# winddori2002/DEX-TTS

Measured on AMD Instinct MI355X. Metric: mel-frames/s at n_timesteps=50, 80-ch mel (sampler only); RTF, higher is better.
Workload: dtype bf16; 1 GPU; gedex_b1: gedex_lj B=1/GPU T=512 n_timesteps=50 (BASELINE.json configs[1]); global_batch=1, frames=512, hipgraph=False, parallelism=1 GPU

## Files before the change

### dex_tts_amd/csrc/dex_api.hip

```cpp
#include <hip/hip_runtime.h>
#include <cstdlib>

#include <cmath>
#include <cstdarg>
#include <atomic>
#include <cstdio>
#include <mutex>
#include <cstring>
#include <map>
#include <unordered_map>
#include <string_view>
#include <string>
#include <vector>

#include "../../include/dex_amd.h"
#include "kernels.h"
#include "weight_store.h"

using namespace dex;

namespace dex {
namespace {
const char* const KNOB_NAMES[] = {
    "DEX_CONV_STREAM", "DEX_CONV_PP", "DEX_CONV_SKIP_DEAD", "DEX_H_BF16", "DEX_ATTN_SEPARATE", "DEX_ATTN_Q64", "DEX_ATTN_Q64_TAIL", "DEX_ATTN_Q64_HALF", "DEX_DIT_XCDS", "DEX_ATTN_GENERIC", "DEX_RES2", "DEX_LP_INTER", "DEX_DIT_CHAIN",
    "DEX_DIT_CLUSTER", "DEX_DIT_CLUSTER_LOCAL", "DEX_ATTN_X_LP", "DEX_RES_X_LP", "DEX_CAT_LP", "DEX_XCD_MAP", "DEX_DEBUG_DROP_HANDOFF", "DEX_PATCH_FUSED",
    "DEX_CONV_DOWN", "DEX_CONVT_UP", "DEX_DEBUG_PLAN",
    "DEX_ATTN_SHARED_W8", "DEX_CONVT_MT", "DEX_CONVT_WGS", "DEX_CONV_DOWN_WGS", "DEX_CONV_REGW", "DEX_CONV_REGW_RES", "DEX_CONV_SMALL_MAX", "DEX_CONV_TH8",
    "DEX_CONV_W8", "DEX_DWCONV_CAP", "DEX_FINAL_CAP", "DEX_FIRST_CAP", "DEX_FIRST_MFMA", "DEX_GEMM_NWALK", "DEX_NWALK_SPLIT", "DEX_NWALK_BM", "DEX_POS_COL", "DEX_POS_COL_MIN",
    "DEX_POS_CT", "DEX_REGW_MIN_TILES", "DEX_REGW_WGS", "DEX_ROWCHAIN64", "DEX_ROWCHAIN64A", "DEX_TIV_CAP", "DEX_TV_CHAIN", "DEX_TIV_FOLD", "DEX_LINATTN_NSUB", "DEX_TV_FOLD", "DEX_OUT2_MIN", "DEX_NWALK_DMA",
    "DEX_LINATTN_HEADWAVES", "DEX_LINATTN_OUT2_HW", "DEX_CONV_ROUND1", "DEX_CONV_RESIDENT", "DEX_KVCTX_ROWS", "DEX_OUT2_ROWS", "DEX_PE_TOK", "DEX_NWALK_SMALL"};
constexpr int N_KNOBS = (int)(sizeof(KNOB_NAMES) / sizeof(KNOB_NAMES[0]));
int knob_parse(const char* e) {
    if (!e) return KNOB_UNSET;
    char* end = nullptr;
    const long v = strtol(e, &end, 10);
    if (end == e) {
        static bool warned = false;
        if (!warned) { warned = true; fprintf(stderr, "libdexamd: ignoring a DEX_* knob whose value '%s' is not an integer\n", e); }
        return KNOB_UNSET;
    }
    return (int)v;
}
struct KnobSnapshot {
    int v[N_KNOBS];
    KnobSnapshot() { for (int i = 0; i < N_KNOBS; ++i) v[i] = knob_parse(getenv(KNOB_NAMES[i])); }
};
thread_local const KnobSnapshot* t_knobs = nullptr;
struct WsplitScope {
    bool prev;
    explicit WsplitScope(bool on) : prev(g_lp_wsplit) { g_lp_wsplit = on; }
    ~WsplitScope() { g_lp_wsplit = prev; }
};
struct KnobScope {
    const KnobSnapshot* prev;
    explicit KnobScope(const KnobSnapshot* k) : prev(t_knobs) { t_knobs = k; }
    ~KnobScope() { t_knobs = prev; }
};
}
static int knob_index(const char* name) {
    static const std::unordered_map<std::string_view, int> idx = [] {
        std::unordered_map<std::string_view, int> m;
        for (int i = 0; i < N_KNOBS; ++i) m.emplace(KNOB_NAMES[i], i);
        return m;
    }();
    const auto it = idx.find(std::string_view(name));
    return it == idx.end() ? -1 : it->second;
}
int knob(const char* name) {
    if (t_knobs) {
        const int i = knob_index(name);
        if (i >= 0) return t_knobs->v[i];
    }
    return knob_parse(getenv(name));
}
}
static_assert(PREC_FP32 == DEX_PREC_FP32 && PREC_BF16 == DEX_PREC_BF16 && PREC_FP16 == DEX_PREC_FP16 && PREC_FP16X2 == DEX_PREC_FP16X2, "kernels.h mirrors DexPrecision");

namespace {
void xcd_map_probe();

struct TD { float* p; int ld; int coff; int C; int lp = 0; };

struct ResW { PackedW w1, w2, wr; const float *b1, *g1, *be1, *b2, *g2, *be2, *br, *mlp_w, *mlp_b; int cin, cout; };
constexpr int ATT_KSPLIT_MAX = 4;
static int att_split_cap(long tokens) { return tokens <= 20480 ? 8 : ATT_KSPLIT_MAX; }
static bool attention_q64_regime(int N, int B) {
    if (N < 1024) return dit_sep64_small_n(N, B) && dit_rowchain64_form(N, B, 0);
    const int ks = attention_q64_ksplit(N, B, att_split_cap((long)B * N));
    const int nt32 = (N + 31) / 32, ng = (nt32 + 7) / 8;
    return 2L * B * ng * ks >= 128;
}
struct LinW { PackedW wqkv; const float *wqkv_raw, *wout_raw, *bias_eff, *g; LpView wkv[3], wq_frag[3]; int C; };
struct DitBlockW { PackedW wqkv, wproj, wfc1, wfc2; const float *bqkv, *bproj, *bfc1, *bfc2, *ada_w, *ada_b; };

struct Prof { std::string name; hipEvent_t a, b; double flops, bytes; };
struct ProfAgg { std::string name; int calls; double ms, flops, bytes; };

struct Arena {
    char* base = nullptr; size_t off = 0, cap = 0; bool dry = true;
    void* take(size_t bytes) {
        off = (off + 255) & ~size_t(255);
        void* p = dry ? nullptr : (void*)(base + off);
        if (!dry && trace) fprintf(stderr, "plan[%d] off %zu bytes %zu\n", trace++, off, bytes);
        off += bytes;
        return p;
    }
    int trace = 0;
    float* f(size_t n) { return (float*)take(n * sizeof(float)); }
};

}

struct DexCtx : WeightStore {
    DexCtx() : WeightStore("") {}
    DexConfig cfg{};
    int lpi() const { return precision == DEX_PREC_FP16X2 ? 2 : precision == DEX_PREC_FP16 ? 1 : 0; }
    int lp_kind() const { return precision == DEX_PREC_BF16 ? 1 : 2; }
    bool lp() const { return precision != DEX_PREC_FP32; }
    bool tuned = true;
    int precision = DEX_PREC_FP32;
    std::vector<std::vector<ResW>> down_res, up_res;
    std::vector<LinW> down_lin, up_lin;
    std::vector<PackedW> down_ds_w;
    std::vector<std::vector<PackedW>> up_us_w;
    std::vector<const float*> down_ds_b, up_us_b;
    const float *fc_w3 = nullptr, *fc_w1 = nullptr;
    PackedW fin_w, pe_pw, fl_w, tv_wk, tv_wv, tv_wl;
    PackedW pos_w;
    const float *fin_b = nullptr, *fin_g = nullptr, *fin_be = nullptr, *fconv_w = nullptr, *fconv_b = nullptr;
    const float *pe_dw = nullptr, *pe_db = nullptr, *pe_pb = nullptr, *pos_b = nullptr, *freq_pos = nullptr;
    std::vector<DitBlockW> blocks;
    const float *fl_b = nullptr, *fl_ada_w = nullptr, *fl_ada_b = nullptr;
    const float *tv_wq_raw = nullptr;
    float *mel_basis = nullptr, *mel_filt = nullptr; void* mel_ws = nullptr; size_t mel_ws_bytes = 0;
    const int* last_xerr = nullptr;
    int* st_host = nullptr; hipEvent_t st_ev = nullptr; bool st_pending = false;
    struct Tap { std::string name; const float* p; std::vector<int64_t> shape; };
    std::vector<Tap> taps;
    bool prof_on = false;
    std::vector<Prof> prof;
    std::vector<ProfAgg> prof_agg;
    struct GraphEntry { std::vector<uint64_t> key; hipGraphExec_t exec; uint64_t stamp; const int* xerr; };
    std::vector<GraphEntry> graphs;
    uint64_t graph_clock = 0;
    void drop_graphs() { for (auto& g : graphs) hipGraphExecDestroy(g.exec); graphs.clear(); }
    template <typename F> int replay(const std::vector<uint64_t>& key, hipStream_t st, F&& enqueue);
    void reset_records() {
        taps.clear();
        if (prof_on) { for (auto& pr : prof) { hipEventDestroy(pr.a); hipEventDestroy(pr.b); } prof.clear(); prof_agg.clear(); }
    }
};

template <typename F> int DexCtx::replay(const std::vector<uint64_t>& key, hipStream_t st, F&& enqueue) {
    GraphEntry* hit = nullptr;
    for (auto& g : graphs) if (g.key == key) { hit = &g; break; }
    if (!hit) {
        constexpr size_t MAX_GRAPHS = 8;
        if (graphs.size() >= MAX_GRAPHS) {
            size_t lru = 0;
            for (size_t i = 1; i < graphs.size(); ++i) if (graphs[i].stamp < graphs[lru].stamp) lru = i;
            hipGraphExecDestroy(graphs[lru].exec);
            graphs.erase(graphs.begin() + lru);
        }
        hipGraph_t graph = nullptr;
        DEX_HIPCHK(this, hipStreamBeginCapture(st, hipStreamCaptureModeThreadLocal));
        const int rc = enqueue();
        hipError_t ec = hipStreamEndCapture(st, &graph);
        if (rc) { if (graph) hipGraphDestroy(graph); return rc; }
        if (ec != hipSuccess || !graph) return fail(DEX_ERR_HIP, "stream capture failed: %s", hipGetErrorString(ec));
        hipGraphExec_t exec = nullptr;
        ec = hipGraphInstantiate(&exec, graph, nullptr, nullptr, 0);
        hipGraphDestroy(graph);
        if (ec != hipSuccess) return fail(DEX_ERR_HIP, "hipGraphInstantiate failed: %s", hipGetErrorString(ec));
        graphs.push_back({key, exec, 0, last_xerr});
        hit = &graphs.back();
    }
    last_xerr = hit->xerr;
    hit->stamp = ++graph_clock;
// ... 1763 lines not shown
```

### dex_tts_amd/csrc/dit_rowchain.hip

```cpp
#include <hip/hip_runtime.h>
#include "kernels.h"
#include <cstdlib>
#include "lp_util.h"
#include "kernels_lp.h"

namespace dex {
namespace DEX_LP_NS {

typedef float f32x16 __attribute__((ext_vector_type(16)));
typedef unsigned short u16;

namespace {

constexpr int RC_H = 256, RC_MLP = 512, RC_ROWS = 32, RC_NW = 8;
constexpr int A_LD = RC_H + 8;
constexpr int H_LD = RC_MLP + 8;
constexpr int X_LD = RC_H + 4;
constexpr int AT_LD = 132;
constexpr size_t RC_LDS_ATTN = (size_t)(RC_NW * 32 * AT_LD + RC_NW * 64) * sizeof(float);
constexpr size_t RC_LDS = (size_t)RC_ROWS * (A_LD + H_LD) * sizeof(u16) + (size_t)RC_ROWS * X_LD * sizeof(float) + 4 * RC_H * sizeof(float);

__device__ __forceinline__ float gelu_erf_rc(float x) {
    const float z = fabsf(x) * 0.70710678118654752440f;
    const float t = __builtin_amdgcn_rcpf(fmaf(0.3275911f, z, 1.0f));
// ... 803 lines not shown
    {
        float4 v[4]; bool ok[4];
#pragma unroll
        for (int k = 0; k < 4; ++k) {
            const int row = wave + 4 * k;
            const bool need_q = row >= 10 || row == 2 || row == 3;
            ok[k] = row < 13 && (need_q ? has_q : !p.qkv_only);
            const float* src = !ok[k] ? ada
                             : row == 0 ? ada + 3 * RC_H : row == 1 ? ada + 4 * RC_H
                             : row == 2 ? p.next_shift + (long)step * p.next_step_stride
                             : row == 3 ? p.next_scale + (long)step * p.next_step_stride
                             : row == 4 ? ada + 2 * RC_H : row == 5 ? p.bp : row == 6 ? ada + 5 * RC_H : row == 7 ? p.b2
                             : row < 10 ? p.b1 + (row - 8) * RC_H : p.bq + (row - 10) * RC_H;
            v[k] = reinterpret_cast<const float4*>(src)[tid & 63];
        }
#pragma unroll
        for (int k = 0; k < 4; ++k) {
            const int row = wave + 4 * k;
            if (row == 1 || row == 3) { v[k].x += 1.f; v[k].y += 1.f; v[k].z += 1.f; v[k].w += 1.f; }
            if (ok[k]) reinterpret_cast<float4*>(PRM + row * RC_H)[tid & 63] = v[k];
        }
    }
    for (;;) {
        const int next = tile + (int)gridDim.x;
        const bool more = next < ntiles;
        RCA_DESC(, tile, true)
        RCA_DESC(_n, more ? next : tile, more)
        const long hb = ((long)b * 2 + (wave >> 1)) * p.Npad * 256;
        const int hsz = has_q ? p.Npad * 256 : 0;
        const auto rq = __builtin_amdgcn_make_buffer_rsrc(reinterpret_cast<unsigned char*>(p.Qh) + hb, 0, hsz, 0x00020000);
        const auto rk = __builtin_amdgcn_make_buffer_rsrc(reinterpret_cast<unsigned char*>(p.Kh) + hb, 0, hsz, 0x00020000);
        const auto rv = __builtin_amdgcn_make_buffer_rsrc(reinterpret_cast<unsigned char*>(p.Vt) + hb, 0, hsz, 0x00020000);
        const long long* dbg = p.dbg ? p.dbg + ((long)tile * 4 + wave) * 32 : nullptr;
#ifdef RCA_TIMING
        if (dbg && (tid & 63) == 0) const_cast<long long*>(dbg)[31] = tile == (int)blockIdx.x ? t_entry : 0;
#endif
        if (p.qkv_only) { asm volatile(RCA_ASM_QKV RCA_OPERANDS); }
        else if (has_q) { asm volatile(RCA_ASM_FULL RCA_OPERANDS); }
        else { asm volatile(RCA_ASM_LAST RCA_OPERANDS); }
        if (!more) break;
        tile = next;
    }
#undef RCA_OPERANDS
#undef RCA_DESC
}

namespace {
constexpr int CL_AH_LD = 128 + 8;
constexpr int CL_RED_LD = 33;
typedef unsigned u32x4v __attribute__((ext_vector_type(4)));

__device__ __forceinline__ void wload8(WT8& w, const void* W, long lo_u4, int ksteps_total, int nt, int ks0, int lane) {
    const uint4* src = reinterpret_cast<const uint4*>(W) + ((long)nt * ksteps_total + ks0) * 64 + lane;
#pragma unroll
    for (int j = 0; j < 8; ++j) w.h[j] = src[j * 64];
#ifdef DEX_LP_WSPLIT
#pragma unroll
    for (int j = 0; j < 8; ++j) w.l[j] = src[lo_u4 + j * 64];
#endif
    __builtin_amdgcn_sched_barrier(0);
}
__device__ __forceinline__ void mma8(f32x16& acc, const WT8& w, const u16* a_lane) {
    u32x4 a[8];
#pragma unroll
    for (int j = 0; j < 8; ++j) a[j] = *reinterpret_cast<const u32x4*>(a_lane + j * 16);
    __builtin_amdgcn_sched_barrier(0);
#pragma unroll
    for (int j = 0; j < 8; ++j) acc = DEX_MFMA_LP(__builtin_bit_cast(lp8, a[j]), __builtin_bit_cast(lp8, w.h[j]), acc, 0, 0, 0);
#ifdef DEX_LP_WSPLIT
#pragma unroll
    for (int j = 0; j < 8; ++j) acc = DEX_MFMA_LP(__builtin_bit_cast(lp8, a[j]), __builtin_bit_cast(lp8, w.l[j]), acc, 0, 0, 0);
#endif
}
__device__ __forceinline__ void ln_regs_to_A(float4 (&v)[4], u16* As, const float* shift, const float* scale, int row, int seg) {
    float4 sc[4], sh[4];
#pragma unroll
    for (int q = 0; q < 4; ++q) {
        sc[q] = *reinterpret_cast<const float4*>(scale + q * 64 + seg * 4);
        sh[q] = *reinterpret_cast<const float4*>(shift + q * 64 + seg * 4);
    }
    float s = 0.f;
#pragma unroll
    for (int q = 0; q < 4; ++q) s += (v[q].x + v[q].y) + (v[q].z + v[q].w);
#pragma unroll
    for (int o = 1; o < 16; o <<= 1) s += __shfl_xor(s, o);
    const float mean = s * (1.f / RC_H);
    float ss = 0.f;
#pragma unroll
    for (int q = 0; q < 4; ++q) {
        v[q].x -= mean; v[q].y -= mean; v[q].z -= mean; v[q].w -= mean;
        ss += v[q].x * v[q].x + v[q].y * v[q].y + v[q].z * v[q].z + v[q].w * v[q].w;
    }
#pragma unroll
    for (int o = 1; o < 16; o <<= 1) ss += __shfl_xor(ss, o);
    const float rstd = rsqrtf(ss * (1.f / RC_H) + 1e-6f);
#pragma unroll
    for (int q = 0; q < 4; ++q) {
        uint2 o;
        o.x = pack2_lp(v[q].x * rstd * (1.f + sc[q].x) + sh[q].x, v[q].y * rstd * (1.f + sc[q].y) + sh[q].y);
        o.y = pack2_lp(v[q].z * rstd * (1.f + sc[q].z) + sh[q].z, v[q].w * rstd * (1.f + sc[q].w) + sh[q].w);
        *reinterpret_cast<uint2*>(As + row * A_LD + q * 64 + seg * 4) = o;
    }
}
template <bool LOCAL> struct ClScope {
    static constexpr int ST_AUX = LOCAL ? 0 : 16, LD_AUX = LOCAL ? 1 : 16;
    static __device__ __forceinline__ unsigned poll(unsigned* p) {
        if constexpr (LOCAL) {
            unsigned v;
            asm volatile("global_atomic_or %0, %1, %2, off sc0\n\ts_waitcnt vmcnt(0)" : "=v"(v) : "v"(p), "v"(0u) : "memory");
            return v;
        } else return __hip_atomic_load(p, __ATOMIC_RELAXED, __HIP_MEMORY_SCOPE_AGENT);
    }
    static __device__ __forceinline__ void st(unsigned* p, unsigned v) {
        if constexpr (LOCAL) __hip_atomic_store(p, v, __ATOMIC_RELAXED, __HIP_MEMORY_SCOPE_WORKGROUP);
        else __hip_atomic_store(p, v, __ATOMIC_RELAXED, __HIP_MEMORY_SCOPE_AGENT);
    }
    static __device__ __forceinline__ unsigned long long ld64(const unsigned long long* p) {
        if constexpr (LOCAL) return __hip_atomic_load(p, __ATOMIC_RELAXED, __HIP_MEMORY_SCOPE_WORKGROUP);
        else return __hip_atomic_load(p, __ATOMIC_RELAXED, __HIP_MEMORY_SCOPE_AGENT);
    }
    static __device__ __forceinline__ void st64(unsigned long long* p, unsigned long long v) {
        if constexpr (LOCAL) __hip_atomic_store(p, v, __ATOMIC_RELAXED, __HIP_MEMORY_SCOPE_WORKGROUP);
        else __hip_atomic_store(p, v, __ATOMIC_RELAXED, __HIP_MEMORY_SCOPE_AGENT);
    }
};
__device__ __forceinline__ unsigned xcc_id() {
    unsigned x;
    asm volatile("s_getreg_b32 %0, hwreg(HW_REG_XCC_ID)" : "=s"(x));
    return x & 15u;
}
template <bool LOCAL>
__device__ __forceinline__ void cluster_wait(unsigned* flags, int member, unsigned epoch, unsigned my_xcc, int tid, int* xerr) {
    if (tid < DIT_CLUSTER && tid != member) {
        long long t0 = wall_clock64(), last = t0;
        unsigned v;
        while (((v = ClScope<LOCAL>::poll(flags + tid)) & 0xffffffu) != epoch) {
            __builtin_amdgcn_s_sleep(LOCAL ? 1 : 2);
            const long long now = wall_clock64();
            if (now - last > 100000LL) t0 = now;
            last = now;
            if (now - t0 > 5000000LL) {
                if (((v = ClScope<LOCAL>::poll(flags + tid)) & 0xffffffu) == epoch) break;
                if (xerr) *xerr = 1;
                v = epoch | (my_xcc << 24);
                break;
            }
        }
        if (LOCAL && (v >> 24) != my_xcc && xerr) *xerr = 2;
    }
    __syncthreads();
}
}

template <bool QKV_ONLY, bool LOCAL = false>
__global__ __launch_bounds__(RC_NW * 64) void dit_rowchain_cluster_kernel(const DitChainP p) {
    using Sc = ClScope<LOCAL>;
    extern __shared__ __attribute__((aligned(16))) unsigned char smem_rc[];
    float* X1 = reinterpret_cast<float*>(smem_rc);
    float* P2 = X1 + RC_ROWS * X_LD;
    float* PRM = P2 + RC_ROWS * X_LD;
    float* RED = PRM + 8 * RC_H;
    u16* As = reinterpret_cast<u16*>(RED + 4 * RC_ROWS * CL_RED_LD);
    u16* Ah = As + RC_ROWS * A_LD;
    u16* QS = Ah + RC_ROWS * CL_AH_LD;
    const int tid = threadIdx.x, lane = tid & 63, wave = tid >> 6;
    const int i = lane & 31, hh = lane >> 5;
    const int N = p.rows_per_batch, tpb = (N + RC_ROWS - 1) / RC_ROWS;
    if (p.xlocal && (int)(blockIdx.x & 7) >= p.xcds) return;
    const int cluster = p.xlocal ? (int)(blockIdx.x & 7) + p.xcds * (int)(blockIdx.x / (8 * DIT_CLUSTER)) : (int)blockIdx.x / DIT_CLUSTER;
    const int member = p.xlocal ? (int)(blockIdx.x >> 3) % DIT_CLUSTER : (int)blockIdx.x % DIT_CLUSTER;
    if (cluster >= p.B * tpb) return;
    const unsigned my_xcc = LOCAL ? xcc_id() : 0u;
    const unsigned flagv = p.epoch | (my_xcc << 24);
    const int b = cluster / tpb, n0 = (cluster - b * tpb) * RC_ROWS;
    const long mb = (long)b * N;
    const int step = p.step + b * p.row_bstride;
    const float* ada = p.ada + (long)step * 6 * RC_H;
    const bool has_q = p.next_shift != nullptr;
    float* slab = p.xslab + (long)cluster * DIT_CLUSTER_SLAB_FLOATS;
    unsigned* flags = p.xflag + (long)cluster * DIT_CLUSTER_FLAG_WORDS;
    const __amdgpu_buffer_rsrc_t srs = __builtin_amdgcn_make_buffer_rsrc(slab, 0, (unsigned)(DIT_CLUSTER_SLAB_FLOATS * 4), 0x00020000);
    constexpr unsigned SLAB_B = (32 * 256 + 256) * 4;
    const int row = tid >> 4, seg = tid & 15;
    const int nrow = min(n0 + row, N - 1);

#ifdef DEX_TIMING
    long long cts[16] = {0,0,0,0,0,0,0,0,0,0,0,0,0,0,0,0};
    cts[0] = wall_clock64();
#endif
    float4 prm;
    {
        const int which = tid >> 6, c4 = (tid & 63) * 4;
        const float* src = which == 0 ? ada + 3 * RC_H : which == 1 ? ada + 4 * RC_H
                         : which == 2 ? (has_q ? p.next_shift + (long)step * p.next_step_stride : ada)
                         : which == 3 ? (has_q ? p.next_scale + (long)step * p.next_step_stride : ada)
                         : which == 4 ? ada + 2 * RC_H : which == 5 ? (QKV_ONLY ? ada : p.bp) : which == 6 ? ada + 5 * RC_H : (QKV_ONLY ? ada : p.b2);
        prm = *reinterpret_cast<const float4*>(src + c4);
    }
    float4 xr[4];
#pragma unroll
    for (int q = 0; q < 4; ++q) xr[q] = *reinterpret_cast<const float4*>(p.X + (mb + nrow) * RC_H + q * 64 + seg * 4);

    WT8 w8;
    f32x16 acc;
    if constexpr (!QKV_ONLY) {
        const int head = member >> 1, half = member & 1;
        f32x16 ao[4];
        float am = -INFINITY, al = 0.f;
        {
            union DFr { uint4 u; lp8 v; };
            const long hbq = ((long)b * 2 + head) * p.Npad * 16;
            const uint4* Qg = reinterpret_cast<const uint4*>(p.Qin) + hbq + lane;
            const uint4* Kg = reinterpret_cast<const uint4*>(p.Kin) + hbq + lane;
            const uint4* Vg = reinterpret_cast<const uint4*>(p.Vin) + hbq + lane;
            const int ntiles = (N + 31) / 32;
            const int t_lo = half ? (ntiles + 1) / 2 : 0, t_hi = half ? ntiles : (ntiles + 1) / 2;
            DFr qf[8], kf[8], vf[4][2];
            int kt = t_lo + wave;
            {
                const uint4* qp = Qg + (long)(n0 >> 5) * 512;
#pragma unroll
                for (int ks = 0; ks < 8; ++ks) qf[ks].u = qp[ks * 64];
                const long t0 = min(kt, ntiles - 1);
                const uint4* kp = Kg + t0 * 512;
#pragma unroll
                for (int ks = 0; ks < 8; ++ks) kf[ks].u = kp[ks * 64];
                const uint4* vp = Vg + t0 * 512;
#pragma unroll
                for (int t = 0; t < 4; ++t)
#pragma unroll
                    for (int k2 = 0; k2 < 2; ++k2) vf[t][k2].u = vp[(t * 2 + k2) * 64];
            }
#pragma unroll
            for (int t = 0; t < 4; ++t)
#pragma unroll
                for (int r = 0; r < 16; ++r) ao[t][r] = 0.f;
            while (kt < t_hi) {
                const int k0 = kt * 32, kn = kt + RC_NW;
                f32x16 sc;
#pragma unroll
                for (int r = 0; r < 16; ++r) sc[r] = 0.f;
#pragma unroll
                for (int ks = 0; ks < 8; ++ks) sc = DEX_MFMA_LP(kf[ks].v, qf[ks].v, sc, 0, 0, 0);
                if (kn < t_hi) {
                    const uint4* kp = Kg + (long)kn * 512;
#pragma unroll
                    for (int ks = 0; ks < 8; ++ks) kf[ks].u = kp[ks * 64];
                }
                if (k0 + 32 > N) {
#pragma unroll
                    for (int r = 0; r < 16; ++r) if (k0 + (r & 3) + 8 * (r >> 2) + 4 * hh >= N) sc[r] = -INFINITY;
                }
                float mx = -INFINITY;
#pragma unroll
                for (int r = 0; r < 16; ++r) mx = fmaxf(mx, sc[r]);
                mx = fmaxf(mx, __shfl_xor(mx, 32));
                if (__builtin_amdgcn_ballot_w64(mx > am + 8.f) != 0) {
                    const float m_new = fmaxf(am, mx);
                    const float alpha = exp2f(am - m_new);
                    al *= alpha;
                    am = m_new;
#pragma unroll
                    for (int t = 0; t < 4; ++t)
#pragma unroll
                        for (int r = 0; r < 16; ++r) ao[t][r] *= alpha;
                }
                float psum = 0.f;
#pragma unroll
                for (int r = 0; r < 16; ++r) { sc[r] = __builtin_amdgcn_exp2f(sc[r] - am); psum += sc[r]; }
                al += psum;
#pragma unroll
                for (int k2 = 0; k2 < 2; ++k2) {
                    DFr pb;
                    pb.u.x = pack2_lp(sc[8 * k2 + 0], sc[8 * k2 + 1]); pb.u.y = pack2_lp(sc[8 * k2 + 2], sc[8 * k2 + 3]);
                    pb.u.z = pack2_lp(sc[8 * k2 + 4], sc[8 * k2 + 5]); pb.u.w = pack2_lp(sc[8 * k2 + 6], sc[8 * k2 + 7]);
#pragma unroll
                    for (int t = 0; t < 4; ++t) ao[t] = DEX_MFMA_LP(vf[t][k2].v, pb.v, ao[t], 0, 0, 0);
                }
                if (kn < t_hi) {
                    const uint4* vp = Vg + (long)kn * 512;
#pragma unroll
                    for (int t = 0; t < 4; ++t)
#pragma unroll
                        for (int k2 = 0; k2 < 2; ++k2) vf[t][k2].u = vp[(t * 2 + k2) * 64];
                }
                kt = kn;
            }
            al += __shfl_xor(al, 32);
        }
#ifdef DEX_TIMING
    cts[1] = wall_clock64();
#endif
        wload8(w8, p.Wp, LO_WP, 16, wave, 8 * head, lane);
        float* scr = reinterpret_cast<float*>(smem_rc);
        {
            float* oS = scr + wave * (32 * AT_LD);
#pragma unroll
            for (int t = 0; t < 4; ++t)
#pragma unroll
                for (int rq = 0; rq < 4; ++rq)
                    *reinterpret_cast<float4*>(oS + i * AT_LD + t * 32 + 8 * rq + 4 * hh) =
                        make_float4(ao[t][rq * 4 + 0], ao[t][rq * 4 + 1], ao[t][rq * 4 + 2], ao[t][rq * 4 + 3]);
            if (hh == 0) { scr[RC_NW * 32 * AT_LD + (wave * 2 + 0) * 32 + i] = am; scr[RC_NW * 32 * AT_LD + (wave * 2 + 1) * 32 + i] = al; }
        }
        lds_barrier();
        float myM, myL;
        float4 ov[2];
        {
            const float* stat = scr + RC_NW * 32 * AT_LD;
            float mw[RC_NW], M = -INFINITY;
#pragma unroll
            for (int w = 0; w < RC_NW; ++w) { mw[w] = stat[(w * 2) * 32 + row]; M = fmaxf(M, mw[w]); }
            float L = 0.f, f[RC_NW];
#pragma unroll
            for (int w = 0; w < RC_NW; ++w) { f[w] = (mw[w] == -INFINITY) ? 0.f : exp2f(mw[w] - M); L += f[w] * stat[(w * 2 + 1) * 32 + row]; }
            const float inv = L > 0.f ? 1.f / L : 0.f;
#pragma unroll
            for (int qq = 0; qq < 2; ++qq) {
                float4 a = make_float4(0.f, 0.f, 0.f, 0.f);
#pragma unroll
                for (int w = 0; w < RC_NW; ++w) {
                    const float4 t4 = *reinterpret_cast<const float4*>(scr + (w * 32 + row) * AT_LD + qq * 64 + seg * 4);
                    a.x = fmaf(f[w], t4.x, a.x); a.y = fmaf(f[w], t4.y, a.y); a.z = fmaf(f[w], t4.z, a.z); a.w = fmaf(f[w], t4.w, a.w);
                }
                ov[qq] = make_float4(a.x * inv, a.y * inv, a.z * inv, a.w * inv);
            }
            myM = M; myL = L;
        }
        lds_barrier();
#pragma unroll
        for (int qq = 0; qq < 2; ++qq) {
            uint2 o;
            o.x = pack2_lp(ov[qq].x, ov[qq].y); o.y = pack2_lp(ov[qq].z, ov[qq].w);
            *reinterpret_cast<uint2*>(Ah + row * CL_AH_LD + qq * 64 + seg * 4) = o;
        }
        *reinterpret_cast<float4*>(PRM + (tid >> 6) * RC_H + (tid & 63) * 4) = prm;
        lds_barrier();

#ifdef DEX_TIMING
    cts[2] = wall_clock64();
#endif
        acc = zero16();
        mma8(acc, w8, Ah + i * CL_AH_LD + hh * 8);
        wload8(w8, p.W1, LO_W1, 16, 4 * member + (wave & 3), 8 * (wave >> 2), lane);
        const int col = wave * 32 + i;
#pragma unroll
        for (int r = 0; r < 16; ++r) X1[((r & 3) + 8 * (r >> 2) + 4 * hh) * X_LD + col] = acc[r];
        lds_barrier();

#ifdef DEX_TIMING
    cts[3] = wall_clock64();
#endif
        {
            const unsigned base = (0 * DIT_CLUSTER + member) * SLAB_B;
#pragma unroll
            for (int q = 0; q < 4; ++q) {
                const float4 v = *reinterpret_cast<const float4*>(X1 + row * X_LD + q * 64 + seg * 4);
                const u32x4v u = {__float_as_uint(v.x), __float_as_uint(v.y), __float_as_uint(v.z), __float_as_uint(v.w)};
                __builtin_amdgcn_raw_buffer_store_b128(u, srs, base + (unsigned)(q * 512 + tid) * 16u, 0, Sc::ST_AUX);
            }
            if (seg == 0) {
                const unsigned long long ml = (unsigned long long)__float_as_uint(myM) | ((unsigned long long)__float_as_uint(myL) << 32);
                Sc::st64(reinterpret_cast<unsigned long long*>(slab + (0 * DIT_CLUSTER + member) * (SLAB_B / 4) + 32 * 256) + row, ml);
            }
            asm volatile("s_waitcnt vmcnt(0)" ::: "memory");
            __syncthreads();
            if (tid == 0 && !(p.xdrop == 1 && member == 3)) Sc::st(flags + 0 * DIT_CLUSTER + member, flagv);
        }

#ifdef DEX_TIMING
    cts[4] = wall_clock64();
#endif
        cluster_wait<LOCAL>(flags + 0 * DIT_CLUSTER, member, p.epoch, my_xcc, tid, p.xerr);
#ifdef DEX_TIMING
    cts[5] = wall_clock64();
#endif

        {
            u32x4v pv[DIT_CLUSTER][4];
            float pm[DIT_CLUSTER], pl[DIT_CLUSTER];
#pragma unroll
            for (int c = 0; c < DIT_CLUSTER; ++c) {
                if (c == member) continue;
                const unsigned base = (0 * DIT_CLUSTER + c) * SLAB_B;
#pragma unroll
                for (int q = 0; q < 4; ++q) pv[c][q] = __builtin_amdgcn_raw_buffer_load_b128(srs, base + (unsigned)(q * 512 + tid) * 16u, 0, Sc::LD_AUX);
                const unsigned long long ml = Sc::ld64(reinterpret_cast<const unsigned long long*>(slab + (0 * DIT_CLUSTER + c) * (SLAB_B / 4) + 32 * 256) + row);
                pm[c] = __uint_as_float((unsigned)ml); pl[c] = __uint_as_float((unsigned)(ml >> 32));
            }
            pm[member] = myM; pl[member] = myL;
            float wgt[DIT_CLUSTER];
#pragma unroll
            for (int h = 0; h < 2; ++h) {
                const float M = fmaxf(pm[2 * h], pm[2 * h + 1]);
                const float fa = pl[2 * h] > 0.f ? pl[2 * h] * exp2f(pm[2 * h] - M) : 0.f, fb = pl[2 * h + 1] > 0.f ? pl[2 * h + 1] * exp2f(pm[2 * h + 1] - M) : 0.f;
                const float inv = 1.f / (fa + fb);
                wgt[2 * h] = fa * inv; wgt[2 * h + 1] = fb * inv;
            }
            float4 v[4];
#pragma unroll
            for (int q = 0; q < 4; ++q) {
                const float4 own = *reinterpret_cast<const float4*>(X1 + row * X_LD + q * 64 + seg * 4);
                float4 sacc = make_float4(0.f, 0.f, 0.f, 0.f);
#pragma unroll
                for (int c = 0; c < DIT_CLUSTER; ++c) {
                    const float4 pc = c == member ? own : make_float4(__uint_as_float(pv[c][q].x), __uint_as_float(pv[c][q].y), __uint_as_float(pv[c][q].z), __uint_as_float(pv[c][q].w));
                    sacc.x = fmaf(wgt[c], pc.x, sacc.x); sacc.y = fmaf(wgt[c], pc.y, sacc.y); sacc.z = fmaf(wgt[c], pc.z, sacc.z); sacc.w = fmaf(wgt[c], pc.w, sacc.w);
                }
                const float4 g = *reinterpret_cast<const float4*>(PRM + 4 * RC_H + q * 64 + seg * 4);
                const float4 bb = *reinterpret_cast<const float4*>(PRM + 5 * RC_H + q * 64 + seg * 4);
                v[q] = make_float4(xr[q].x + g.x * (sacc.x + bb.x), xr[q].y + g.y * (sacc.y + bb.y), xr[q].z + g.z * (sacc.z + bb.z), xr[q].w + g.w * (sacc.w + bb.w));
                *reinterpret_cast<float4*>(X1 + row * X_LD + q * 64 + seg * 4) = v[q];
            }
            ln_regs_to_A(v, As, PRM, PRM + RC_H, row, seg);
        }

#ifdef DEX_TIMING
    cts[6] = wall_clock64();
#endif
        lds_barrier();
#ifdef DEX_TIMING
    cts[7] = wall_clock64();
#endif

        {
            const int ct = wave & 3, kh = wave >> 2;
            acc = zero16();
            mma8(acc, w8, As + i * A_LD + hh * 8 + kh * 128);
            wload8(w8, p.W2, LO_W2, 32, wave, 8 * member, lane);
            if (kh == 1) {
#pragma unroll
                for (int r = 0; r < 16; ++r) RED[(ct * 32 + (r & 3) + 8 * (r >> 2) + 4 * hh) * CL_RED_LD + i] = acc[r];
            }
            lds_barrier();
            if (kh == 0) {
                const float b1v = p.b1[128 * member + ct * 32 + i];
#pragma unroll
                for (int r = 0; r < 16; ++r) {
                    const int rr = (r & 3) + 8 * (r >> 2) + 4 * hh;
                    Ah[rr * CL_AH_LD + ct * 32 + i] = (u16)(pack2_lp(gelu_erf_rc(acc[r] + RED[(ct * 32 + rr) * CL_RED_LD + i] + b1v), 0.f) & 0xffffu);
                }
            }
            lds_barrier();
        }

#ifdef DEX_TIMING
    cts[8] = wall_clock64();
#endif
        acc = zero16();
        mma8(acc, w8, Ah + i * CL_AH_LD + hh * 8);
#pragma unroll
        for (int r = 0; r < 16; ++r) P2[((r & 3) + 8 * (r >> 2) + 4 * hh) * X_LD + col] = acc[r];

#ifdef DEX_TIMING
    cts[9] = wall_clock64();
#endif
        lds_barrier();
        {
            const unsigned base = (1 * DIT_CLUSTER + member) * SLAB_B;
#pragma unroll
            for (int q = 0; q < 4; ++q) {
                const float4 v = *reinterpret_cast<const float4*>(P2 + row * X_LD + q * 64 + seg * 4);
                const u32x4v u = {__float_as_uint(v.x), __float_as_uint(v.y), __float_as_uint(v.z), __float_as_uint(v.w)};
                __builtin_amdgcn_raw_buffer_store_b128(u, srs, base + (unsigned)(q * 512 + tid) * 16u, 0, Sc::ST_AUX);
            }
            asm volatile("s_waitcnt vmcnt(0)" ::: "memory");
            __syncthreads();
            if (tid == 0 && !(p.xdrop == 1 && member == 3)) Sc::st(flags + 1 * DIT_CLUSTER + member, flagv);
        }

#ifdef DEX_TIMING
    cts[10] = wall_clock64();
#endif
        cluster_wait<LOCAL>(flags + 1 * DIT_CLUSTER, member, p.epoch, my_xcc, tid, p.xerr);
#ifdef DEX_TIMING
    cts[11] = wall_clock64();
#endif

        {
            u32x4v pv[DIT_CLUSTER][4];
#pragma unroll
            for (int c = 0; c < DIT_CLUSTER; ++c) {
                if (c == member) continue;
                const unsigned base = (1 * DIT_CLUSTER + c) * SLAB_B;
#pragma unroll
                for (int q = 0; q < 4; ++q) pv[c][q] = __builtin_amdgcn_raw_buffer_load_b128(srs, base + (unsigned)(q * 512 + tid) * 16u, 0, Sc::LD_AUX);
            }
#pragma unroll
            for (int q = 0; q < 4; ++q) {
                const float4 own = *reinterpret_cast<const float4*>(P2 + row * X_LD + q * 64 + seg * 4);
                float4 sacc = make_float4(0.f, 0.f, 0.f, 0.f);
#pragma unroll
                for (int c = 0; c < DIT_CLUSTER; ++c) {
                    const float4 pc = c == member ? own : make_float4(__uint_as_float(pv[c][q].x), __uint_as_float(pv[c][q].y), __uint_as_float(pv[c][q].z), __uint_as_float(pv[c][q].w));
                    sacc.x += pc.x; sacc.y += pc.y; sacc.z += pc.z; sacc.w += pc.w;
                }
                const float4 g = *reinterpret_cast<const float4*>(PRM + 6 * RC_H + q * 64 + seg * 4);
                const float4 bb = *reinterpret_cast<const float4*>(PRM + 7 * RC_H + q * 64 + seg * 4);
                const float4 x1 = *reinterpret_cast<const float4*>(X1 + row * X_LD + q * 64 + seg * 4);
                const float4 x2 = make_float4(x1.x + g.x * (sacc.x + bb.x), x1.y + g.y * (sacc.y + bb.y), x1.z + g.z * (sacc.z + bb.z), x1.w + g.w * (sacc.w + bb.w));
                xr[q] = x2;
                if (q == member && n0 + row < N) *reinterpret_cast<float4*>(p.X + (mb + n0 + row) * RC_H + q * 64 + seg * 4) = x2;
            }
        }

#ifdef DEX_TIMING
    cts[12] = wall_clock64();
#endif
        if (!has_q) return;
    } else {
        *reinterpret_cast<float4*>(PRM + (tid >> 6) * RC_H + (tid & 63) * 4) = prm;
        lds_barrier();
    }
    WT16 wq;
    const int nt = 6 * member + wave;
    if (wave < 6) wload(wq, p.Wq, LO_WQ, 16, nt, 0, lane);
    ln_regs_to_A(xr, As, PRM + 2 * RC_H, PRM + 3 * RC_H, row, seg);
    lds_barrier();

#ifdef DEX_TIMING
    cts[13] = wall_clock64();
#endif
    if (wave < 6) {
        acc = zero16();
        if (nt < 16) {
            const QkvBias qb = qkv_bias<0>(p, nt, lane);
            mma16t(acc, wq, As + i * A_LD + hh * 8);
            if (nt < 8) store_qkv_tile_d<0>(p, acc, qb, nt, b, n0, lane); else store_qkv_tile_d<1>(p, acc, qb, nt, b, n0, lane);
        } else {
            const QkvBias qb = qkv_bias<2>(p, nt, lane);
            mma16(acc, wq, As + i * A_LD + hh * 8);
            store_qkv_tile_d<2>(p, acc, qb, nt, b, n0, lane);
        }
    }
#ifdef DEX_TIMING
    cts[14] = wall_clock64();
    if (p.dbg && tid == 0) for (int q = 0; q < 16; ++q) p.dbg[blockIdx.x * 16 + q] = cts[q];
#endif
}
constexpr size_t RC_LDS_CLUSTER_CHAIN = (size_t)(2 * RC_ROWS * X_LD + 8 * RC_H + 4 * RC_ROWS * CL_RED_LD) * sizeof(float)
                                        + (size_t)(RC_ROWS * A_LD + RC_ROWS * CL_AH_LD + RC_NW * RC_ROWS * QK_LD) * sizeof(u16);
constexpr size_t RC_LDS_CLUSTER = RC_LDS_CLUSTER_CHAIN > RC_LDS_ATTN ? RC_LDS_CLUSTER_CHAIN : RC_LDS_ATTN;

bool dit_rowchain_cluster_form(int rows_per_batch, int B) {
#if defined(DEX_LP_WSPLIT) && !defined(DEX_WS_HAVE_RCC)
    return false;
#endif
   
    const int on = knob_or("DEX_DIT_CLUSTER", 1);
    return on && (long)B * ((rows_per_batch + RC_ROWS - 1) / RC_ROWS) * DIT_CLUSTER <= 256;
}

bool dit_rowchain_cluster_local_fits(int rows_per_batch, int B) {
    const int on = knob_or("DEX_DIT_CLUSTER_LOCAL", 1);
    const long tiles = (long)B * ((rows_per_batch + RC_ROWS - 1) / RC_ROWS);
    return on && dit_rowchain_cluster_form(rows_per_batch, B) && (tiles + 7) / 8 * 8 * DIT_CLUSTER <= 256;
}
int dit_rowchain_cluster_xcds(int rows_per_batch, int B) {
    const long tiles = (long)B * ((rows_per_batch + RC_ROWS - 1) / RC_ROWS);
    const int forced = knob_or("DEX_DIT_XCDS", 0);
    int x = forced >= 1 && forced <= 8 ? forced : 8;
    while (x < 8 && (tiles + x - 1) / x * DIT_CLUSTER > 32) ++x;
    return x;
}

bool dit_rowchain_supported(int hidden, int mlp_hidden) {
#if defined(DEX_LP_WSPLIT) && !defined(DEX_WS_HAVE_RC)
    return false;
#endif
    return hidden == RC_H && mlp_hidden == RC_MLP; }
bool dit_rowchain64_form(int rows_per_batch, int B, int attn_inline) {
#if defined(DEX_LP_WSPLIT) && !defined(DEX_WS_HAVE_RC64)
    return false;
#endif
   
    const int m64 = knob_or("DEX_ROWCHAIN64", 1);
    const long wg32 = (long)B * ((rows_per_batch + RC_ROWS - 1) / RC_ROWS);
    const bool small_n = dit_sep64_small_n(rows_per_batch, B);
    return m64 && !attn_inline && (m64 == 2 || wg32 >= 768 || small_n);
}

void launch_dit_rowchain(const DitChainP& p, hipStream_t st) {
    if (p.xslab && (p.attn_inline || p.qkv_only) && dit_rowchain_cluster_form(p.rows_per_batch, p.B)) {
        static bool attrc = false;
        if (!attrc) {
            hipFuncSetAttribute(reinterpret_cast<const void*>(&dit_rowchain_cluster_kernel<false, false>), hipFuncAttributeMaxDynamicSharedMemorySize, (int)RC_LDS_CLUSTER);
            hipFuncSetAttribute(reinterpret_cast<const void*>(&dit_rowchain_cluster_kernel<false, true>), hipFuncAttributeMaxDynamicSharedMemorySize, (int)RC_LDS_CLUSTER);
            hipFuncSetAttribute(reinterpret_cast<const void*>(&dit_rowchain_cluster_kernel<true, false>), hipFuncAttributeMaxDynamicSharedMemorySize, (int)RC_LDS_CLUSTER);
            attrc = true;
        }
        const int tiles = p.B * ((p.rows_per_batch + RC_ROWS - 1) / RC_ROWS);
        const int xc = p.xlocal ? (p.xcds >= 1 && p.xcds <= 8 ? p.xcds : 8) : 8;
        const dim3 gridc((p.xlocal ? (tiles + xc - 1) / xc * 8 : tiles) * DIT_CLUSTER);
        if (p.qkv_only) {
            g_last_symbol = "dit_rowchain_cluster_kernel<true,false>";
            hipLaunchKernelGGL((dit_rowchain_cluster_kernel<true, false>), gridc, dim3(RC_NW * 64), RC_LDS_CLUSTER, st, p);
        } else if (p.xdrop == 2) {
            DitChainP q = p; q.xlocal = 0;
            g_last_symbol = "dit_rowchain_cluster_kernel<false,true>";
            hipLaunchKernelGGL((dit_rowchain_cluster_kernel<false, true>), dim3(tiles * DIT_CLUSTER), dim3(RC_NW * 64), RC_LDS_CLUSTER, st, q);
        } else if (p.xlocal) {
            g_last_symbol = "dit_rowchain_cluster_kernel<false,true>";
            hipLaunchKernelGGL((dit_rowchain_cluster_kernel<false, true>), gridc, dim3(RC_NW * 64), RC_LDS_CLUSTER, st, p);
        } else {
            g_last_symbol = "dit_rowchain_cluster_kernel<false,false>";
            hipLaunchKernelGGL((dit_rowchain_cluster_kernel<false, false>), gridc, dim3(RC_NW * 64), RC_LDS_CLUSTER, st, p);
        }
        return;
    }
    static bool attr = false;
    if (!attr) {
        hipFuncSetAttribute(reinterpret_cast<const void*>(&dit_rowchain_kernel<false>), hipFuncAttributeMaxDynamicSharedMemorySize, (int)RC_LDS);
        hipFuncSetAttribute(reinterpret_cast<const void*>(&dit_rowchain_kernel<true>), hipFuncAttributeMaxDynamicSharedMemorySize,
                            (int)(RC_LDS_ATTN > RC_LDS ? RC_LDS_ATTN : RC_LDS));
        attr = true;
    }
    {
        if (dit_rowchain64_form(p.rows_per_batch, p.B, p.attn_inline)) {
            static bool attr64 = false;
            if (!attr64) {
                hipFuncSetAttribute(reinterpret_cast<const void*>(&dit_rowchain64_kernel), hipFuncAttributeMaxDynamicSharedMemorySize, (int)RC64_LDS);
                attr64 = true;
            }
            if (knob_or("DEX_ROWCHAIN64A", 1) && p.row_bstride == 0 && (p.qkv_only || (p.o_lp && p.ksplit <= 1 && p.tail_ks <= 1))) {
                static bool attr64a = false;
                if (!attr64a) {
                    hipFuncSetAttribute(reinterpret_cast<const void*>(&dit_rowchain64a_kernel), hipFuncAttributeMaxDynamicSharedMemorySize, (int)RCA_LDS_BYTES);
                    attr64a = true;
                }
                g_last_symbol = "dit_rowchain64a_kernel";
                const int ncu = device_cus();
                const int ntiles = p.B * ((p.rows_per_batch + 63) / 64);
                hipLaunchKernelGGL(dit_rowchain64a_kernel, dim3(ntiles < ncu ? ntiles : ncu), dim3(256), RCA_LDS_BYTES, st, p);
                return;
            }
            g_last_symbol = "dit_rowchain64_kernel";
            hipLaunchKernelGGL(dit_rowchain64_kernel, dim3(p.B * ((p.rows_per_batch + 63) / 64)), dim3(RC_NW * 64), RC64_LDS, st, p);
            return;
        }
    }
    dim3 grid(p.B * ((p.rows_per_batch + RC_ROWS - 1) / RC_ROWS));
    if (p.attn_inline && !p.qkv_only) {
        DitChainP q = p;
        q.xcd_map = (p.B % 8 == 0 && !knob_off("DEX_XCD_MAP")) ? 1 : 0;
        g_last_symbol = q.xcd_map ? "dit_rowchain_kernel<true> xcd_map=1" : "dit_rowchain_kernel<true> xcd_map=0";
        hipLaunchKernelGGL(dit_rowchain_kernel<true>, grid, dim3(RC_NW * 64), RC_LDS_ATTN > RC_LDS ? RC_LDS_ATTN : RC_LDS, st, q);
    }
    else {
        g_last_symbol = "dit_rowchain_kernel<false>";
        hipLaunchKernelGGL(dit_rowchain_kernel<false>, grid, dim3(RC_NW * 64), RC_LDS, st, p);
    }
}

__global__ void pack_lp_frag_kernel(const float* __restrict__ src, u16* __restrict__ dst, int K, int N) {
    const long total = (long)K * N;
    for (long o = (long)blockIdx.x * blockDim.x + threadIdx.x; o < total; o += (long)gridDim.x * blockDim.x) {
        const int j = (int)(o & 7), lane = (int)((o >> 3) & 63);
        const long t = o >> 9;
        const int ks = (int)(t % (K / 16)), nt = (int)(t / (K / 16));
        const int k = ks * 16 + (lane >> 5) * 8 + j, n = nt * 32 + (lane & 31);
        dst[o] = (u16)(pack2_lp(src[(long)k * N + n], 0.f) & 0xffffu);
    }
}
__global__ void pack_lp_frag_nk_kernel(const float* __restrict__ src, u16* __restrict__ dst, int K, int N) {
    const long total = (long)K * N;
    for (long o = (long)blockIdx.x * blockDim.x + threadIdx.x; o < total; o += (long)gridDim.x * blockDim.x) {
        const int j = (int)(o & 7), lane = (int)((o >> 3) & 63);
        const long t = o >> 9;
        const int ks = (int)(t % (K / 16)), nt = (int)(t / (K / 16));
        const int k = ks * 16 + (lane >> 5) * 8 + j, n = nt * 32 + (lane & 31);
        dst[o] = (u16)(pack2_lp(src[(long)n * K + k], 0.f) & 0xffffu);
    }
}
void launch_pack_lp_frag_nk(const float* src, void* dst, int K, int N, hipStream_t st) {
    hipLaunchKernelGGL(pack_lp_frag_nk_kernel, dim3(256), dim3(256), 0, st, src, reinterpret_cast<u16*>(dst), K, N);
}
void launch_pack_lp_frag(const float* src, void* dst, int K, int N, hipStream_t st) {
    hipLaunchKernelGGL(pack_lp_frag_kernel, dim3(256), dim3(256), 0, st, src, reinterpret_cast<u16*>(dst), K, N);
}

}
}
```

Measured before the change: 29600 mel-frames/s.

## Prefetch cluster weights before handoff waits and skip own-slab reloads in DiT cluster kernel

Adds a SCHED variant of the DiT cluster rowchain kernel, on by default. It issues the W2, Wq and b1 weight loads before the inter-workgroup cluster_wait barriers so their latency overlaps the wait. In the reduction, each member reads only its peers' slabs and takes its own partial from LDS and registers instead of reloading it from global memory. This costs extra register pressure, since weights and peer partials are held in registers across the barrier, and keeps the old path behind a knob.

```diff
diff --git a/dex_tts_amd/csrc/dex_api.hip b/dex_tts_amd/csrc/dex_api.hip
--- a/dex_tts_amd/csrc/dex_api.hip
+++ b/dex_tts_amd/csrc/dex_api.hip
@@ -23,7 +23,7 @@
 namespace {
 const char* const KNOB_NAMES[] = {
     "DEX_CONV_STREAM", "DEX_CONV_PP", "DEX_CONV_SKIP_DEAD", "DEX_H_BF16", "DEX_ATTN_SEPARATE", "DEX_ATTN_Q64", "DEX_ATTN_Q64_TAIL", "DEX_ATTN_Q64_HALF", "DEX_DIT_XCDS", "DEX_ATTN_GENERIC", "DEX_RES2", "DEX_LP_INTER", "DEX_DIT_CHAIN",
-    "DEX_DIT_CLUSTER", "DEX_DIT_CLUSTER_LOCAL", "DEX_ATTN_X_LP", "DEX_RES_X_LP", "DEX_CAT_LP", "DEX_XCD_MAP", "DEX_DEBUG_DROP_HANDOFF", "DEX_PATCH_FUSED",
+    "DEX_DIT_CLUSTER", "DEX_DIT_CLUSTER_LOCAL", "DEX_DIT_CLUSTER_SCHED", "DEX_ATTN_X_LP", "DEX_RES_X_LP", "DEX_CAT_LP", "DEX_XCD_MAP", "DEX_DEBUG_DROP_HANDOFF", "DEX_PATCH_FUSED",
     "DEX_CONV_DOWN", "DEX_CONVT_UP", "DEX_DEBUG_PLAN",
     "DEX_ATTN_SHARED_W8", "DEX_CONVT_MT", "DEX_CONVT_WGS", "DEX_CONV_DOWN_WGS", "DEX_CONV_REGW", "DEX_CONV_REGW_RES", "DEX_CONV_SMALL_MAX", "DEX_CONV_TH8",
     "DEX_CONV_W8", "DEX_DWCONV_CAP", "DEX_FINAL_CAP", "DEX_FIRST_CAP", "DEX_FIRST_MFMA", "DEX_GEMM_NWALK", "DEX_NWALK_SPLIT", "DEX_NWALK_BM", "DEX_POS_COL", "DEX_POS_COL_MIN",
diff --git a/dex_tts_amd/csrc/dit_rowchain.hip b/dex_tts_amd/csrc/dit_rowchain.hip
--- a/dex_tts_amd/csrc/dit_rowchain.hip
+++ b/dex_tts_amd/csrc/dit_rowchain.hip
@@ -979,7 +979,13 @@
 }
 }
 
-template <bool QKV_ONLY, bool LOCAL = false>
+template <int C, typename T>
+__device__ __forceinline__ T cl_pick(int member, const T& own, const T (&peer)[DIT_CLUSTER - 1]) {
+    return C == member ? own : C < member ? peer[C < DIT_CLUSTER - 1 ? C : DIT_CLUSTER - 2] : peer[C > 0 ? C - 1 : 0];
+}
+typedef unsigned u32x2v __attribute__((ext_vector_type(2)));
+
+template <bool QKV_ONLY, bool LOCAL = false, bool SCHED = true>
 __global__ __launch_bounds__(RC_NW * 64) void dit_rowchain_cluster_kernel(const DitChainP p) {
     using Sc = ClScope<LOCAL>;
     extern __shared__ __attribute__((aligned(16))) unsigned char smem_rc[];
@@ -1029,7 +1035,15 @@
     for (int q = 0; q < 4; ++q) xr[q] = *reinterpret_cast<const float4*>(p.X + (mb + nrow) * RC_H + q * 64 + seg * 4);
 
     WT8 w8;
+    WT16 wq;
+    const int nt = 6 * member + wave;
+    if constexpr (QKV_ONLY && SCHED) {
+        if (wave < 6) wload(wq, p.Wq, LO_WQ, 16, nt, 0, lane);
+    }
     f32x16 acc;
+    WT8 w2;
+    float b1e = 0.f;
+    if constexpr (!QKV_ONLY && SCHED) b1e = p.b1[128 * member + (wave & 3) * 32 + i];
     if constexpr (!QKV_ONLY) {
         const int head = member >> 1, half = member & 1;
         f32x16 ao[4];
@@ -1198,12 +1212,52 @@
 #ifdef DEX_TIMING
     cts[4] = wall_clock64();
 #endif
+        if constexpr (SCHED) wload8(w2, p.W2, LO_W2, 32, wave, 8 * member, lane);
         cluster_wait<LOCAL>(flags + 0 * DIT_CLUSTER, member, p.epoch, my_xcc, tid, p.xerr);
 #ifdef DEX_TIMING
     cts[5] = wall_clock64();
 #endif
 
-        {
+        if constexpr (SCHED) {
+            u32x4v pj[4][DIT_CLUSTER - 1];
+            u32x2v mlj[DIT_CLUSTER - 1];
+#pragma unroll
+            for (int j = 0; j < DIT_CLUSTER - 1; ++j) {
+                const unsigned base = (unsigned)(0 * DIT_CLUSTER + j + (j >= member ? 1 : 0)) * SLAB_B;
+#pragma unroll
+                for (int q = 0; q < 4; ++q) pj[q][j] = __builtin_amdgcn_raw_buffer_load_b128(srs, base + (unsigned)(q * 512 + tid) * 16u, 0, Sc::LD_AUX);
+                mlj[j] = __builtin_amdgcn_raw_buffer_load_b64(srs, base + (unsigned)(32 * 256 * 4 + row * 8), 0, Sc::LD_AUX);
+            }
+            const u32x2v myml = {__float_as_uint(myM), __float_as_uint(myL)};
+            const u32x2v ml[DIT_CLUSTER] = {cl_pick<0>(member, myml, mlj), cl_pick<1>(member, myml, mlj), cl_pick<2>(member, myml, mlj), cl_pick<3>(member, myml, mlj)};
+            float wgt[DIT_CLUSTER];
+#pragma unroll
+            for (int h = 0; h < 2; ++h) {
+                const float ma = __uint_as_float(ml[2 * h].x), la = __uint_as_float(ml[2 * h].y), mb2 = __uint_as_float(ml[2 * h + 1].x), lb = __uint_as_float(ml[2 * h + 1].y);
+                const float M = fmaxf(ma, mb2);
+                const float fa = la > 0.f ? la * exp2f(ma - M) : 0.f, fb = lb > 0.f ? lb * exp2f(mb2 - M) : 0.f;
+                const float inv = 1.f / (fa + fb);
+                wgt[2 * h] = fa * inv; wgt[2 * h + 1] = fb * inv;
+            }
+            float4 v[4];
+#pragma unroll
+            for (int q = 0; q < 4; ++q) {
+                const float4 o4 = *reinterpret_cast<const float4*>(X1 + row * X_LD + q * 64 + seg * 4);
+                const u32x4v own = {__float_as_uint(o4.x), __float_as_uint(o4.y), __float_as_uint(o4.z), __float_as_uint(o4.w)};
+                const u32x4v pc[DIT_CLUSTER] = {cl_pick<0>(member, own, pj[q]), cl_pick<1>(member, own, pj[q]), cl_pick<2>(member, own, pj[q]), cl_pick<3>(member, own, pj[q])};
+                float4 sacc = make_float4(0.f, 0.f, 0.f, 0.f);
+#pragma unroll
+                for (int c = 0; c < DIT_CLUSTER; ++c) {
+                    sacc.x = fmaf(wgt[c], __uint_as_float(pc[c].x), sacc.x); sacc.y = fmaf(wgt[c], __uint_as_float(pc[c].y), sacc.y);
+                    sacc.z = fmaf(wgt[c], __uint_as_float(pc[c].z), sacc.z); sacc.w = fmaf(wgt[c], __uint_as_float(pc[c].w), sacc.w);
+                }
+                const float4 g = *reinterpret_cast<const float4*>(PRM + 4 * RC_H + q * 64 + seg * 4);
+                const float4 bb = *reinterpret_cast<const float4*>(PRM + 5 * RC_H + q * 64 + seg * 4);
+                v[q] = make_float4(xr[q].x + g.x * (sacc.x + bb.x), xr[q].y + g.y * (sacc.y + bb.y), xr[q].z + g.z * (sacc.z + bb.z), xr[q].w + g.w * (sacc.w + bb.w));
+                *reinterpret_cast<float4*>(X1 + row * X_LD + q * 64 + seg * 4) = v[q];
+            }
+            ln_regs_to_A(v, As, PRM, PRM + RC_H, row, seg);
+        } else {
             u32x4v pv[DIT_CLUSTER][4];
             float pm[DIT_CLUSTER], pl[DIT_CLUSTER];
 #pragma unroll
@@ -1254,14 +1308,15 @@
             const int ct = wave & 3, kh = wave >> 2;
             acc = zero16();
             mma8(acc, w8, As + i * A_LD + hh * 8 + kh * 128);
-            wload8(w8, p.W2, LO_W2, 32, wave, 8 * member, lane);
+            if constexpr (SCHED) w8 = w2;
+            else wload8(w8, p.W2, LO_W2, 32, wave, 8 * member, lane);
             if (kh == 1) {
 #pragma unroll
                 for (int r = 0; r < 16; ++r) RED[(ct * 32 + (r & 3) + 8 * (r >> 2) + 4 * hh) * CL_RED_LD + i] = acc[r];
             }
             lds_barrier();
             if (kh == 0) {
-                const float b1v = p.b1[128 * member + ct * 32 + i];
+                const float b1v = SCHED ? b1e : p.b1[128 * member + ct * 32 + i];
 #pragma unroll
                 for (int r = 0; r < 16; ++r) {
                     const int rr = (r & 3) + 8 * (r >> 2) + 4 * hh;
@@ -1299,12 +1354,40 @@
 #ifdef DEX_TIMING
     cts[10] = wall_clock64();
 #endif
+        if constexpr (SCHED) {
+            if (has_q && wave < 6) wload(wq, p.Wq, LO_WQ, 16, nt, 0, lane);
+        }
         cluster_wait<LOCAL>(flags + 1 * DIT_CLUSTER, member, p.epoch, my_xcc, tid, p.xerr);
 #ifdef DEX_TIMING
     cts[11] = wall_clock64();
 #endif
 
-        {
+        if constexpr (SCHED) {
+            u32x4v pj[4][DIT_CLUSTER - 1];
+#pragma unroll
+            for (int j = 0; j < DIT_CLUSTER - 1; ++j) {
+                const unsigned base = (unsigned)(1 * DIT_CLUSTER + j + (j >= member ? 1 : 0)) * SLAB_B;
+#pragma unroll
+                for (int q = 0; q < 4; ++q) pj[q][j] = __builtin_amdgcn_raw_buffer_load_b128(srs, base + (unsigned)(q * 512 + tid) * 16u, 0, Sc::LD_AUX);
+            }
+#pragma unroll
+            for (int q = 0; q < 4; ++q) {
+                const float4 o4 = *reinterpret_cast<const float4*>(P2 + row * X_LD + q * 64 + seg * 4);
+                const u32x4v own = {__float_as_uint(o4.x), __float_as_uint(o4.y), __float_as_uint(o4.z), __float_as_uint(o4.w)};
+                const u32x4v pc[DIT_CLUSTER] = {cl_pick<0>(member, own, pj[q]), cl_pick<1>(member, own, pj[q]), cl_pick<2>(member, own, pj[q]), cl_pick<3>(member, own, pj[q])};
+                float4 sacc = make_float4(0.f, 0.f, 0.f, 0.f);
+#pragma unroll
+                for (int c = 0; c < DIT_CLUSTER; ++c) {
+                    sacc.x += __uint_as_float(pc[c].x); sacc.y += __uint_as_float(pc[c].y); sacc.z += __uint_as_float(pc[c].z); sacc.w += __uint_as_float(pc[c].w);
+                }
+                const float4 g = *reinterpret_cast<const float4*>(PRM + 6 * RC_H + q * 64 + seg * 4);
+                const float4 bb = *reinterpret_cast<const float4*>(PRM + 7 * RC_H + q * 64 + seg * 4);
+                const float4 x1 = *reinterpret_cast<const float4*>(X1 + row * X_LD + q * 64 + seg * 4);
+                const float4 x2 = make_float4(x1.x + g.x * (sacc.x + bb.x), x1.y + g.y * (sacc.y + bb.y), x1.z + g.z * (sacc.z + bb.z), x1.w + g.w * (sacc.w + bb.w));
+                xr[q] = x2;
+                if (q == member && n0 + row < N) *reinterpret_cast<float4*>(p.X + (mb + n0 + row) * RC_H + q * 64 + seg * 4) = x2;
+            }
+        } else {
             u32x4v pv[DIT_CLUSTER][4];
 #pragma unroll
             for (int c = 0; c < DIT_CLUSTER; ++c) {
@@ -1339,9 +1422,9 @@
         *reinterpret_cast<float4*>(PRM + (tid >> 6) * RC_H + (tid & 63) * 4) = prm;
         lds_barrier();
     }
-    WT16 wq;
-    const int nt = 6 * member + wave;
-    if (wave < 6) wload(wq, p.Wq, LO_WQ, 16, nt, 0, lane);
+    if constexpr (!SCHED) {
+        if (wave < 6) wload(wq, p.Wq, LO_WQ, 16, nt, 0, lane);
+    }
     ln_regs_to_A(xr, As, PRM + 2 * RC_H, PRM + 3 * RC_H, row, seg);
     lds_barrier();
 
@@ -1411,27 +1494,33 @@
     if (p.xslab && (p.attn_inline || p.qkv_only) && dit_rowchain_cluster_form(p.rows_per_batch, p.B)) {
         static bool attrc = false;
         if (!attrc) {
-            hipFuncSetAttribute(reinterpret_cast<const void*>(&dit_rowchain_cluster_kernel<false, false>), hipFuncAttributeMaxDynamicSharedMemorySize, (int)RC_LDS_CLUSTER);
-            hipFuncSetAttribute(reinterpret_cast<const void*>(&dit_rowchain_cluster_kernel<false, true>), hipFuncAttributeMaxDynamicSharedMemorySize, (int)RC_LDS_CLUSTER);
-            hipFuncSetAttribute(reinterpret_cast<const void*>(&dit_rowchain_cluster_kernel<true, false>), hipFuncAttributeMaxDynamicSharedMemorySize, (int)RC_LDS_CLUSTER);
+            for (const void* f : {reinterpret_cast<const void*>(&dit_rowchain_cluster_kernel<false, false, true>), reinterpret_cast<const void*>(&dit_rowchain_cluster_kernel<false, true, true>),
+                                  reinterpret_cast<const void*>(&dit_rowchain_cluster_kernel<true, false, true>), reinterpret_cast<const void*>(&dit_rowchain_cluster_kernel<false, false, false>),
+                                  reinterpret_cast<const void*>(&dit_rowchain_cluster_kernel<false, true, false>), reinterpret_cast<const void*>(&dit_rowchain_cluster_kernel<true, false, false>)})
+                hipFuncSetAttribute(f, hipFuncAttributeMaxDynamicSharedMemorySize, (int)RC_LDS_CLUSTER);
             attrc = true;
         }
         const int tiles = p.B * ((p.rows_per_batch + RC_ROWS - 1) / RC_ROWS);
         const int xc = p.xlocal ? (p.xcds >= 1 && p.xcds <= 8 ? p.xcds : 8) : 8;
         const dim3 gridc((p.xlocal ? (tiles + xc - 1) / xc * 8 : tiles) * DIT_CLUSTER);
+        const bool sched = knob_or("DEX_DIT_CLUSTER_SCHED", 1) != 0;
         if (p.qkv_only) {
-            g_last_symbol = "dit_rowchain_cluster_kernel<true,false>";
-            hipLaunchKernelGGL((dit_rowchain_cluster_kernel<true, false>), gridc, dim3(RC_NW * 64), RC_LDS_CLUSTER, st, p);
+            g_last_symbol = sched ? "dit_rowchain_cluster_kernel<true,false>" : "dit_rowchain_cluster_kernel<true,false> sched=0";
+            if (sched) hipLaunchKernelGGL((dit_rowchain_cluster_kernel<true, false, true>), gridc, dim3(RC_NW * 64), RC_LDS_CLUSTER, st, p);
+            else hipLaunchKernelGGL((dit_rowchain_cluster_kernel<true, false, false>), gridc, dim3(RC_NW * 64), RC_LDS_CLUSTER, st, p);
         } else if (p.xdrop == 2) {
             DitChainP q = p; q.xlocal = 0;
-            g_last_symbol = "dit_rowchain_cluster_kernel<false,true>";
-            hipLaunchKernelGGL((dit_rowchain_cluster_kernel<false, true>), dim3(tiles * DIT_CLUSTER), dim3(RC_NW * 64), RC_LDS_CLUSTER, st, q);
+            g_last_symbol = sched ? "dit_rowchain_cluster_kernel<false,true>" : "dit_rowchain_cluster_kernel<false,true> sched=0";
+            if (sched) hipLaunchKernelGGL((dit_rowchain_cluster_kernel<false, true, true>), dim3(tiles * DIT_CLUSTER), dim3(RC_NW * 64), RC_LDS_CLUSTER, st, q);
+            else hipLaunchKernelGGL((dit_rowchain_cluster_kernel<false, true, false>), dim3(tiles * DIT_CLUSTER), dim3(RC_NW * 64), RC_LDS_CLUSTER, st, q);
         } else if (p.xlocal) {
-            g_last_symbol = "dit_rowchain_cluster_kernel<false,true>";
-            hipLaunchKernelGGL((dit_rowchain_cluster_kernel<false, true>), gridc, dim3(RC_NW * 64), RC_LDS_CLUSTER, st, p);
+            g_last_symbol = sched ? "dit_rowchain_cluster_kernel<false,true>" : "dit_rowchain_cluster_kernel<false,true> sched=0";
+            if (sched) hipLaunchKernelGGL((dit_rowchain_cluster_kernel<false, true, true>), gridc, dim3(RC_NW * 64), RC_LDS_CLUSTER, st, p);
+            else hipLaunchKernelGGL((dit_rowchain_cluster_kernel<false, true, false>), gridc, dim3(RC_NW * 64), RC_LDS_CLUSTER, st, p);
         } else {
-            g_last_symbol = "dit_rowchain_cluster_kernel<false,false>";
-            hipLaunchKernelGGL((dit_rowchain_cluster_kernel<false, false>), gridc, dim3(RC_NW * 64), RC_LDS_CLUSTER, st, p);
+            g_last_symbol = sched ? "dit_rowchain_cluster_kernel<false,false>" : "dit_rowchain_cluster_kernel<false,false> sched=0";
+            if (sched) hipLaunchKernelGGL((dit_rowchain_cluster_kernel<false, false, true>), gridc, dim3(RC_NW * 64), RC_LDS_CLUSTER, st, p);
+            else hipLaunchKernelGGL((dit_rowchain_cluster_kernel<false, false, false>), gridc, dim3(RC_NW * 64), RC_LDS_CLUSTER, st, p);
         }
         return;
     }
```

New measurement: 29720 mel-frames/s (median of 4 runs). About the same (+0.4%).
